# cvjena/semantic-embeddings

Hardware: AMD Instinct MI355X
Metric: retrieval_Mpairs_per_sec (higher is better)
Workload: dtype f32

## Files before the change

semantic-embeddings_amd/csrc/rank_rows.hip:

```cpp
#include "se_common.h"
#include <stdlib.h>
#include <atomic>
#include <type_traits>

namespace se {

constexpr int RK_THREADS = 512;
constexpr int RK_WAVES = RK_THREADS / WAVE;
constexpr int RK_ITEMS = 16;
constexpr int RK_TILE = RK_THREADS * RK_ITEMS;
constexpr int RK_WCHUNK = RK_TILE / RK_WAVES;
constexpr int RK_NB = 256;

struct RankLds {
    uint32_t gbase[4][RK_NB];
    uint32_t wcnt[RK_WAVES][RK_NB];
    uint32_t tile_start[RK_NB];
    uint32_t wave_tot[RK_WAVES];
    uint32_t tkeys[RK_TILE];
    uint32_t tidx[RK_TILE];
};

__device__ __forceinline__ uint32_t wave_excl_scan(uint32_t v, uint32_t &total)
{
// ... 131 lines not shown
                    }
                    if (valid) {
                        const int rnk = __popcll(peers & lt_mask);
                        const int npeers = __popcll(peers);
                        const uint32_t base = cur[dgt];
                        if (rnk == npeers - 1) cur[dgt] = base + (uint32_t)npeers;
                        L.tkeys[base + rnk] = key[s];
                        L.tidx[base + rnk] = idx[s];
                    }
                }
                wg_barrier();

#pragma unroll
                for (int j = 0; j < RK_ITEMS; j++) {
                    const int i = j * RK_THREADS + tid;
                    if (i < tcount) {
                        const uint32_t k = L.tkeys[i];
                        const uint32_t id = L.tidx[i];
                        const uint32_t d = (k >> shift) & 0xFF;
                        const uint32_t gpos = L.gbase[p][d] + ((uint32_t)i - L.tile_start[d]);
                        if (last) {
                            if (IDX64) ((int64_t *)rank)[row * ldr + gpos] = (int64_t)id;
                            else ((int32_t *)rank)[row * ldr + gpos] = (int32_t)id;
                        } else {
                            dk[gpos] = k;
                            di[gpos] = id;
                        }
                    }
                }
                wg_barrier();
                if (tid < RK_NB) L.gbase[p][tid] += my_total;
            }
        }
    }
}


constexpr int RR_THREADS = 512;
constexpr int RR_WAVES = RR_THREADS / WAVE;
constexpr int RR_SCAN_THREADS = 512;
constexpr int RR_SCAN_WAVES = RR_SCAN_THREADS / WAVE;
static_assert((53248 + RR_THREADS - 1) / RR_THREADS <= 104, "rows of up to 53,248 columns: 104 keys per thread");
constexpr int RR_G = 8;
constexpr int RR_MAX_N = 53248;

__device__ __forceinline__ void differ_mask(uint32_t d, uint32_t &lo, uint32_t &hi)
{
    lo = 0;
    hi = 0;
#pragma unroll
    for (int bb = 0; bb < 8; bb += 2) {
        uint32_t s0 = (uint32_t)__builtin_amdgcn_sbfe((int)d, bb, 1);
        uint32_t s1 = (uint32_t)__builtin_amdgcn_sbfe((int)d, bb + 1, 1);
        asm volatile("" : "+v"(s0), "+v"(s1));
        const uint64_t m0 = __ballot(s0 != 0), m1 = __ballot(s1 != 0);
        lo = __builtin_amdgcn_bitop3_b32(lo, (uint32_t)m0, s0, 0xF6);
        hi = __builtin_amdgcn_bitop3_b32(hi, (uint32_t)(m0 >> 32), s0, 0xF6);
        lo = __builtin_amdgcn_bitop3_b32(lo, (uint32_t)m1, s1, 0xF6);
        hi = __builtin_amdgcn_bitop3_b32(hi, (uint32_t)(m1 >> 32), s1, 0xF6);
    }
}

constexpr uint32_t RR_KEY_NAN = 0xFF900000u;
__device__ __forceinline__ uint32_t rr_pad_key(uint32_t lane) { return 0xFFA00000u + ((lane % 6u) << 20) + (lane << 11) + lane; }
__device__ __forceinline__ uint32_t rr_key(uint32_t u, bool pad, uint32_t pad_key)
{
    const uint32_t sx = (uint32_t)((int32_t)u >> 31);
    uint32_t k = __builtin_amdgcn_bitop3_b32(u, sx, 0x80000000u, 0x1E);
    k -= sx;
    const float f = __uint_as_float(u);
    k = (f != f) ? RR_KEY_NAN : k;
    return pad ? pad_key : k;
}

__device__ __forceinline__ int32_t rr_clamp_i32(int32_t x, int32_t lo, int32_t hi) { return min(max(x, lo), hi); }

template <typename T>
__device__ __forceinline__ void opaque(T &x) { asm volatile("" : "+v"(x)); }

__device__ __forceinline__ uint32_t lds_off(const void *p) { return (uint32_t)(uintptr_t)p; }
__device__ __forceinline__ void lds_wait() { asm volatile("s_waitcnt lgkmcnt(0)" ::: "memory"); }
__device__ __forceinline__ void lds_st16_lo(uint32_t addr, uint32_t v) { asm volatile("ds_write_b16 %0, %1" ::"v"(addr), "v"(v) : "memory"); }
__device__ __forceinline__ void lds_st16_hi(uint32_t addr, uint32_t v) { asm volatile("ds_write_b16_d16_hi %0, %1" ::"v"(addr), "v"(v) : "memory"); }
template <int OFF>
__device__ __forceinline__ void lds_ld16(uint32_t &dst, uint32_t addr) { asm volatile("ds_read_u16 %0, %1 offset:%2" : "=v"(dst) : "v"(addr), "n"(OFF) : "memory"); }
template <int K>
__device__ __forceinline__ void lds_wait_le(uint32_t &landed) { asm volatile("s_waitcnt lgkmcnt(%1)" : "+v"(landed) : "n"(K) : "memory"); }

constexpr int RR_RING = 12;
template <int ITEMS, bool HI, int I = 0>
struct RRRead {
    static __device__ __forceinline__ void run(uint32_t (&a)[ITEMS], uint32_t (&t)[RR_RING], uint32_t addr)
    {
        constexpr int D = RR_RING - 1;
        if constexpr (I < ITEMS) lds_ld16<I * WAVE * 2>(t[I % RR_RING], addr);
        if constexpr (I >= D) {
            constexpr int J = I - D;
            constexpr int newest = (I < ITEMS ? I : ITEMS - 1);
            lds_wait_le<newest - J>(t[J % RR_RING]);
            a[J] = __builtin_amdgcn_perm(t[J % RR_RING], a[J], HI ? 0x05040100u : 0x03020504u);
        }
        if constexpr (I + 1 < ITEMS + D) RRRead<ITEMS, HI, I + 1>::run(a, t, addr);
    }
};

template <int ITEMS, int V, int S0, int I = 0>
struct RRRankFinish {
    static __device__ __forceinline__ void run(uint32_t (&ir)[ITEMS], uint32_t (&key)[ITEMS], uint32_t (&rnk)[V], uint32_t (&base)[V])
    {
        lds_wait_le<2 * (V - 1 - I) + 1>(base[I]);
        ir[S0 + I] = (ir[S0 + I] & 0xFFFF0000u) | (base[I] + rnk[I]);
        opaque(ir[S0 + I]);
        opaque(key[S0 + I]);
        if constexpr (I + 1 < V) RRRankFinish<ITEMS, V, S0, I + 1>::run(ir, key, rnk, base);
    }
};

template <int ITEMS, int S0 = 0>
struct RRRank {
    static __device__ __forceinline__ void run(uint32_t (&ir)[ITEMS], uint32_t (&key)[ITEMS], int shift, int lane, uint32_t cb)
    {
        constexpr int V = (ITEMS - S0 < RR_G) ? (ITEMS - S0) : RR_G;
        static_assert(2 * V - 1 <= 15, "lgkmcnt counts to 15");
        uint32_t rnk[V], base[V];
#pragma unroll
        for (int g = 0; g < V; g++) {
            const uint32_t d = (key[S0 + g] >> shift) & 0xFFu;
            uint32_t dlo, dhi;
            differ_mask(d, dlo, dhi);
            rnk[g] = (uint32_t)lane - __builtin_amdgcn_mbcnt_hi(dhi, __builtin_amdgcn_mbcnt_lo(dlo, 0u));
            const uint32_t ca = cb + (d << 2);
            asm volatile("ds_read_b32 %0, %1" : "=v"(base[g]) : "v"(ca) : "memory");
            if (rnk[g] == 0) {
                const uint32_t np = 64u - (uint32_t)(__popc(dlo) + __popc(dhi));
                asm volatile("ds_add_u32 %0, %1" ::"v"(ca), "v"(np) : "memory");
            }
        }
        RRRankFinish<ITEMS, V, S0>::run(ir, key, rnk, base);
        __builtin_amdgcn_sched_barrier(0);
        if constexpr (S0 + V < ITEMS) RRRank<ITEMS, S0 + V>::run(ir, key, shift, lane, cb);
    }
};

typedef int rr_i32x4 __attribute__((ext_vector_type(4)));
typedef long long rr_i64x2 __attribute__((ext_vector_type(2)));
constexpr int RR_GH = 8;
constexpr int RR_HW_BITS = 11;
constexpr int RR_WIDE_WORDS = 2048;
constexpr uint32_t RR_TWO_SPAN = (1u << 24) - 3u;
constexpr int RR_TWO_OUT = 256;
constexpr int RR_IMG_RUN = 8;
constexpr int RR_IMG_WL = 3072;
constexpr int RR_IMG_MAX_ITEMS = 98;
constexpr uint32_t RR_IMG_NAN_PADHI = 0xFF0u;
template <int ITEMS, bool PEEL, int S = 0>
struct RRRankHW {
    static __device__ __forceinline__ void run(uint32_t (&ir)[ITEMS], uint32_t (&key)[ITEMS], uint32_t (&r)[RR_GH], uint32_t (&sh)[RR_GH],
                                               uint32_t (&grp)[RR_GH], uint32_t shift, uint32_t hshift, uint32_t wlo, uint32_t whi, uint32_t cb,
                                               int lane, bool peel)
    {
        constexpr int SLOT = S % RR_GH;
        uint32_t ca = 0, inc = 0, shv = 0, g = 0xFFFFFFFFu;
        uint64_t part = ~0ull;
        if constexpr (S < ITEMS) {
            const uint32_t w = __builtin_amdgcn_ubfe(key[S], shift, wlo);
            const uint32_t h = __builtin_amdgcn_ubfe(key[S], hshift, whi);
// ... 78 lines not shown
    constexpr int NB = 1 << BITS;
    constexpr int NPASS = (32 + BITS - 1) / BITS;
    constexpr int CNT_WORDS = HWORD ? NB / 2 : NB;
    constexpr bool WIDE = HWORD && ((size_t)RR_THREADS * ITEMS * sizeof(uint16_t) >= (size_t)RR_WAVES * RR_WIDE_WORDS * sizeof(uint32_t));
    constexpr bool IMG = WIDE && VAR == 3;
    constexpr bool RAWKEYS = IMG || (WIDE && VAR == 2);
    static_assert(VAR != 3 || (WIDE && ITEMS <= RR_IMG_MAX_ITEMS && !SEG), "image path: long-row instantiations with room for the tag plane");
    uint32_t *wcnt = reinterpret_cast<uint32_t *>(rr_raw);
    uint32_t *wave_tot = reinterpret_cast<uint32_t *>(rr_raw + rr_region0_bytes<ITEMS, HWORD, VAR>());
    uint16_t *xbuf = reinterpret_cast<uint16_t *>(wave_tot + 32);
    [[maybe_unused]] uint8_t *tagb = rr_raw;
    [[maybe_unused]] uint32_t *wlist = reinterpret_cast<uint32_t *>(rr_raw + (size_t)RR_THREADS * ITEMS + 32);
    [[maybe_unused]] uint32_t *ictl = wave_tot + 24;
    const int tid = threadIdx.x, lane = tid & 63, wave = tid >> 6;
    [[maybe_unused]] const int wave_s = __builtin_amdgcn_readfirstlane(wave);
    const int wpos0 = wave * (ITEMS * WAVE) + lane;
    const uint32_t xb = lds_off(xbuf);
    const uint32_t rb = xb + 2u * (uint32_t)wpos0;
#define RR_DST(IR) (xb + (((IR) & 0xFFFFu) << 1))
    auto row_ptr = [&](int64_t v) -> const float * {
        if constexpr (SEG) return pdist + (v >> seg.shift) * ldp + (v & ((1 << seg.shift) - 1)) * (int64_t)seg.seg_n;
        else return pdist + v * ldp;
    };
    auto row_len = [&](int64_t v) -> int {
        if constexpr (SEG) {
            const int rest = N - (int)(v & ((1 << seg.shift) - 1)) * seg.seg_n;
            return rest < seg.seg_n ? rest : seg.seg_n;
        } else return N;
    };
    uint32_t t_acc[12] = {0, 0, 0, 0, 0, 0, 0, 0, 0, 0, 0, 0}, t_last = PROF ? (uint32_t)__builtin_amdgcn_s_memtime() : 0;
#define RR_T(i) if constexpr (PROF) { const uint32_t now = (uint32_t)__builtin_amdgcn_s_memtime(); t_acc[i] += now - t_last; t_last = now; } else { asm volatile("" ::: "memory"); __builtin_amdgcn_sched_barrier(0); }

    uint32_t key[ITEMS], ir[ITEMS];
    __amdgpu_buffer_rsrc_t ld_rsrc;
    uint32_t ld_voff = 0;
    uint32_t ring[RR_RING];
#define RR_LOAD_ONE(DROW, WPOS, S, NN)                                                                               \
    {                                                                                                                 \
        if ((S) % 16 == 0) {                                                                                          \
            if ((S) == 0) {                                                                                           \
                ld_rsrc = __builtin_amdgcn_make_buffer_rsrc(const_cast<float *>(DROW), 0, (NN) * 4, 0x00020000);     \
                ld_voff = (uint32_t)(WPOS) * 4u;                                                                      \
            } else ld_voff += 4096u;                                                                                  \
            opaque(ld_voff);                                                                                          \
        }                                                                                                             \
        key[S] = (uint32_t)__builtin_amdgcn_raw_buffer_load_b32(ld_rsrc, (int)ld_voff + ((S) % 16) * 256, 0, 0);      \
    }
#define RR_CANON(NN)                                                                                                  \
    {                                                                                                                 \
        int wpos_ = wpos0;                                                                                            \
        opaque(wpos_);                                                                                                \
        const uint32_t pk_ = rr_pad_key((uint32_t)wpos_ & 63u);                                                       \
        _Pragma("unroll") for (int s = 0; s < ITEMS; s++) {                                                           \
            const int pos = wpos_ + s * WAVE;                                                                         \
            key[s] = rr_key(key[s], pos >= (NN), pk_ + (ITEMS <= 88 ? (uint32_t)((((s >> 3) & 7) << 17) | ((s & 7) << 6)) : 0u));  \
        }                                                                                                             \
    }
#define RR_PREFETCH_NEXT_ROW() RR_PREFETCH_NEXT_ROW_IF(end >= 32 && more)
#define RR_PREFETCH_NEXT_ROW_IF(COND) \
    if (COND) { \
                const char *nrow = (const char *)row_ptr(row + gridDim.x); \
                const uint32_t row_bytes = (uint32_t)row_len(row + gridDim.x) * 4u; \
                for (uint32_t off = (uint32_t)tid * 128u; off < row_bytes; off += RR_THREADS * 128u) \
                    asm volatile("global_load_dword %0, %1, off" : "=v"(pf_sink) : "v"(nrow + off) : "memory"); \
            }
#define RR_STREAM_PLANE(P, ROW)                                                                                       \
    {                                                                                                                 \
        uint16_t *pl = seg.planes + (P) * seg.plane_elems + (ROW) * (int64_t)(RR_THREADS * ITEMS);                    \
        int j = tid * 8;                                                                                              \
        opaque(j);                                                                                                    \
        _Pragma("unroll 2") for (; j < RR_THREADS * ITEMS; j += RR_THREADS * 8)                                       \
            *reinterpret_cast<uint4 *>(pl + j) = *reinterpret_cast<const uint4 *>(xbuf + j);                          \
    }
    constexpr int RR_PADS = ITEMS < 8 ? ITEMS : 8;
#define RR_PAD_LOOP(NROW, BODY)                                                                                       \
    {                                                                                                                 \
        const int first_pad_ = ((NROW) - wave_s * (ITEMS * WAVE)) >> 6;    \
        if (first_pad_ >= ITEMS - RR_PADS) {                                                                          \
            _Pragma("unroll") for (int s = ITEMS - RR_PADS; s < ITEMS; s++) { BODY }                                  \
        } else {                                                                                                      \
            _Pragma("unroll") for (int s = 0; s < ITEMS; s++) { BODY }                                                \
        }                                                                                                             \
    }
    if ((int64_t)blockIdx.x < Q) {
        const float *drow = row_ptr(blockIdx.x);
        const int n0 = row_len(blockIdx.x);
        int wpos = wpos0;
        opaque(wpos);
#pragma unroll
        for (int s = 0; s < ITEMS; s++) RR_LOAD_ONE(drow, wpos, s, n0)
        if constexpr (!RAWKEYS) RR_CANON(n0)
    }
    uint32_t pf_sink = 0;
    [[maybe_unused]] int img_level = 0;
    [[maybe_unused]] bool img_again = false;
    [[maybe_unused]] int img_skip0 = 0, img_pen0 = 0, img_skip1 = 0, img_pen1 = 0;
    for (int64_t row = blockIdx.x; row < Q;) {
        const bool more = row + gridDim.x < Q;
        [[maybe_unused]] const int n_next = row_len(more ? row + gridDim.x : row);
        constexpr bool SKIP_WAVES = HWORD && ITEMS <= 88;
        const bool wave_live = !SKIP_WAVES || wave * (ITEMS * WAVE) < row_len(row);
        bool two = false;
        [[maybe_unused]] int n_out = 0;
        if constexpr (IMG) {
            const int n_row = row_len(row);
            if (!img_again) {
                if (img_skip1 > 0) { img_level = 2; img_skip1--; }
                else if (img_skip0 > 0) { img_level = 1; img_skip0--; }
                else img_level = 0;
            }
            bool attempt = img_level < 2;
            uint32_t cbits = 0, base = 0;
            if (attempt) {
                uint32_t mb = 0;
#pragma unroll
                for (int s = 0; s + 1 < ITEMS; s += 2) mb = max(max(mb, key[s] & 0x7FFFFFFFu), key[s + 1] & 0x7FFFFFFFu);
                if constexpr (ITEMS & 1) mb = max(mb, key[ITEMS - 1] & 0x7FFFFFFFu);
#pragma unroll
                for (int off = 32; off > 0; off >>= 1) mb = max(mb, (uint32_t)__shfl_xor((int)mb, off, 64));
                if (lane == 0) wave_tot[wave] = mb;
                wg_barrier();
                if (tid == 0) { ictl[0] = 0; ictl[1] = 0; }
#pragma unroll
                for (int w = 0; w < RR_WAVES; w++) mb = max(mb, wave_tot[w]);
                mb = (uint32_t)__builtin_amdgcn_readfirstlane((int)mb);
                const uint32_t e = (mb >> 23) + ((mb & 0x7FFFFFu) > 0x400000u ? 1u : 0u) - (img_level == 0 ? 1u : 0u);
                two = mb >= 0x0D800000u && mb < 0x7E800000u;
                cbits = (e + 1u) << 23;
                base = e << 23;
            }
            if (two) {
                const float c = __uint_as_float(cbits);
                int wpos_ = wpos0;
                opaque(wpos_);
                const uint32_t pk_ = ((RR_IMG_NAN_PADHI + ((uint32_t)wpos_ & 15u)) << 20) | (((uint32_t)wpos_ & 63u) << 14);
                const uint32_t tb = lds_off(tagb) + (uint32_t)wpos_;
#pragma unroll
                for (int s = 0; s < ITEMS; s++) {
                    const uint32_t t = __float_as_uint(__uint_as_float(key[s]) + c);
                    const uint32_t q = (uint32_t)rr_clamp_i32(__builtin_elementwise_sub_sat((int32_t)t, (int32_t)base), 0, 0xFEFFFF);
                    asm volatile("ds_write_b8 %0, %1 offset:%2" ::"v"(tb), "v"(q), "n"(s * WAVE) : "memory");
                    key[s] = q << 8;
                }
                if (wave_s * (ITEMS * WAVE) + ITEMS * WAVE > n_row) {
                    RR_PAD_LOOP(n_row, key[s] = (wpos_ + s * WAVE >= n_row) ? pk_ : key[s];)
                }
            } else {
                RR_CANON(n_row)
            }
            RR_T(8)
        }
        if constexpr (WIDE && VAR == 2) {
            uint32_t *stat = wave_tot;
            uint2 *outl = reinterpret_cast<uint2 *>(wcnt);
            const int n_row = row_len(row);
            int32_t mxi = 0;
            uint32_t umx = 0;
#pragma unroll
            for (int s = 0; s + 1 < ITEMS; s += 2) {
                mxi = max(max(mxi, rr_clamp_i32((int32_t)key[s], 0, 0x7F800000)), rr_clamp_i32((int32_t)key[s + 1], 0, 0x7F800000));
                umx = max(max(umx, key[s]), key[s + 1]);
            }
            if constexpr (ITEMS & 1) { mxi = max(mxi, rr_clamp_i32((int32_t)key[ITEMS - 1], 0, 0x7F800000)); umx = max(umx, key[ITEMS - 1]); }
            mxi = umx > 0xFF800000u ? 0x7F800000 : mxi;
#pragma unroll
            for (int off = 32; off > 0; off >>= 1) mxi = max(mxi, __shfl_xor(mxi, off, 64));
            if (lane == 0) stat[wave] = (uint32_t)mxi;
            if (tid == 0) stat[2 * RR_WAVES] = 0;
            RR_T(9)
            wg_barrier();
            RR_T(10)
#pragma unroll
            for (int w = 0; w < RR_WAVES; w++) mxi = max(mxi, (int32_t)stat[w]);
            const int32_t kmax = __builtin_amdgcn_readfirstlane(mxi);
            const int32_t lo = kmax > (int32_t)RR_TWO_SPAN ? kmax - (int32_t)RR_TWO_SPAN : 1, lo1 = lo - 1;
            uint32_t below_l = 0;
            {
                int wpos = wpos0;
                opaque(wpos);
#pragma unroll
                for (int s = 0; s < ITEMS; s++) below_l += ((int32_t)key[s] < lo) ? 1u : 0u;
                if (wave_s * (ITEMS * WAVE) + ITEMS * WAVE > n_row) {
                    int32_t lo_b = lo;
                    opaque(lo_b);
// ... 92 lines not shown
                    ex += c;
                }
            }
            } else {
                const bool scanner = tid < RR_SCAN_THREADS;
                const int st = scanner ? tid : 0;
                uint32_t T0 = 0, T1 = 0, U0 = 0, U1 = 0;
#pragma unroll
                for (int w = 0; w < RR_WAVES; w++) {
                    const uint2 v = *reinterpret_cast<const uint2 *>(pcnt + w * pcw + 2 * st);
                    T0 += v.x; T1 += v.y;
                }
                if (wide) {
                    __builtin_amdgcn_sched_barrier(0);
#pragma unroll
                    for (int w = 0; w < RR_WAVES; w++) {
                        const uint2 v = *reinterpret_cast<const uint2 *>(pcnt + w * pcw + CNT_WORDS + 2 * st);
                        U0 += v.x; U1 += v.y;
                    }
                    __builtin_amdgcn_sched_barrier(0);
                }
                uint32_t wtot, wtot2 = 0, ex2 = 0;
                uint32_t ex = wave_excl_scan(T0 + T1, wtot);
                if (wide) ex2 = wave_excl_scan(U0 + U1, wtot2);
                if (scanner && lane == 63) { wave_tot[wave] = wtot; wave_tot[RR_SCAN_WAVES + wave] = wtot2; }
                wg_barrier();
                uint32_t all = 0, all2 = 0;
#pragma unroll
                for (int w = 0; w < RR_SCAN_WAVES; w++) {
                    const uint32_t wt = wave_tot[w], wt2 = wave_tot[RR_SCAN_WAVES + w];
                    all += wt; all2 += wt2;
                    ex += (w < wave) ? wt : 0u;
                    ex2 += (w < wave) ? wt2 : 0u;
                }
                ex2 += all;
                const uint32_t hi = (all + all2) << 16;
                ex += hi; ex2 += hi;
                if (scanner) {
                uint32_t s0 = ex, s1 = ex + T0;
#pragma unroll
                for (int w = 0; w < RR_WAVES; w++) {
                    uint2 *wp = reinterpret_cast<uint2 *>(pcnt + w * pcw + 2 * tid);
                    const uint2 v = *wp;
                    *wp = make_uint2(s0, s1);
                    s0 += v.x; s1 += v.y;
                }
                if (wide) {
                    __builtin_amdgcn_sched_barrier(0);
                    s0 = ex2; s1 = ex2 + U0;
#pragma unroll
                    for (int w = 0; w < RR_WAVES; w++) {
                        uint2 *wp = reinterpret_cast<uint2 *>(pcnt + w * pcw + CNT_WORDS + 2 * tid);
                        const uint2 v = *wp;
                        *wp = make_uint2(s0, s1);
                        s0 += v.x; s1 += v.y;
                    }
                }
                }
            }
            wg_barrier();
            RR_T(2)
            if (!(IMG && two)) { RR_PREFETCH_NEXT_ROW() }
            if (wave_live) {
#pragma unroll
            for (int s0 = 0; s0 < ITEMS; s0 += 8) {
                uint32_t first[8];
#pragma unroll
                for (int g = 0; g < 8; g++)
                    if (s0 + g < ITEMS) {
                        if constexpr (HWORD) first[g] = reinterpret_cast<const uint16_t *>(mycnt)[(__builtin_amdgcn_ubfe(key[s0 + g], (uint32_t)shift, wlo) << 1) | __builtin_amdgcn_ubfe(key[s0 + g], hshift, whi)];
                        else first[g] = mycnt[(key[s0 + g] >> shift) & 0xFFu];
                    }
#pragma unroll
                for (int g = 0; g < 8; g++)
                    if (s0 + g < ITEMS) {
                        ir[s0 + g] += first[g];
                        opaque(ir[s0 + g]);
                    }
                __builtin_amdgcn_sched_barrier(0);
            }
            }
            if (wide) wg_barrier();
            RR_T(3)
            if (wave_live) {
#pragma unroll
                for (int s = 0; s < ITEMS; s++) { opaque(ir[s]); lds_st16_hi(RR_DST(ir[s]), ir[s]); }
            }
            lds_wait();
            wg_barrier();
            RR_T(4)
            const bool last = end >= 32;
            if (last) {
                if constexpr (!SEG) break;
                else {
                    RR_STREAM_PLANE(0, row)
                    wg_barrier();
                }
            } else {
                if (wave_live) RRRead<ITEMS, true>::run(ir, ring, rb);
                lds_wait();
                wg_barrier();
            }
            RR_T(5)
            if (wave_live) {
#pragma unroll
                for (int s = 0; s < ITEMS; s++) { opaque(ir[s]); lds_st16_hi(RR_DST(ir[s]), key[s]); }
            }
            lds_wait();
            wg_barrier();
            if (SEG && last) {
                RR_STREAM_PLANE(1, row)
            } else {
                if (wave_live) RRRead<ITEMS, true>::run(key, ring, rb);
                lds_wait();
            }
            if (end < 16 || SEG) {
                wg_barrier();
                if (wave_live) {
#pragma unroll
                    for (int s = 0; s < ITEMS; s++) { opaque(ir[s]); lds_st16_lo(RR_DST(ir[s]), key[s]); }
                }
                lds_wait();
                wg_barrier();
                if (SEG && last) break;
                if (wave_live) RRRead<ITEMS, false>::run(key, ring, rb);
                lds_wait();
            }
            RR_T(6)
        }
#undef RR_DST
        if constexpr (WIDE && VAR == 2) {
            if (two && n_out > 1) {
                const uint2 *outl = reinterpret_cast<const uint2 *>(wcnt);
                if (tid < n_out) {
                    const uint2 me = outl[tid];
                    int r = 0;
                    for (int j = 0; j < n_out; j++) {
                        const uint2 o = outl[j];
                        r += (o.x < me.x || (o.x == me.x && o.y < me.y)) ? 1 : 0;
                    }
                    xbuf[r] = (uint16_t)me.y;
                }
                wg_barrier();
            }
        }
        [[maybe_unused]] bool img_fail = false;
        if constexpr (IMG) {
            const float *drow = row_ptr(more ? row + gridDim.x : row);
            int wpos = wpos0;
            opaque(wpos);
#pragma unroll
            for (int s = 0; s < ITEMS; s++) RR_LOAD_ONE(drow, wpos, s, n_next)
        }
        if constexpr (IMG) {
            if (two) {
                int n_row = row_len(row);
                int tsc = wave_s * WAVE + (int)__builtin_amdgcn_mbcnt_hi(~0u, __builtin_amdgcn_mbcnt_lo(~0u, 0u));
                opaque(n_row);
                opaque(tsc);
                const float *drow_cur = row_ptr(row);
                constexpr int NS = RR_THREADS * ITEMS;
                constexpr int NG = (NS / 8 + RR_THREADS - 1) / RR_THREADS;
                uint32_t S[NG];
                uint32_t nstart = 0;
                uint4 xg[NG];
                uint32_t nxg[NG];
#pragma unroll
                for (int g = 0; g < NG; g++) {
                    const int b0 = (tsc + RR_THREADS * g) * 8;
                    const int bs = b0 < n_row - 1 ? b0 : 0;
                    xg[g] = *reinterpret_cast<const uint4 *>(xbuf + bs);
                    nxg[g] = xbuf[bs + 8 < NS ? bs + 8 : bs];
                }
                constexpr int TD = 1;
                uint32_t t[TD + 1][9];
                auto tag_reads = [&](int g, uint32_t (&tt)[9]) {
                    const uint32_t xi[4] = {xg[g].x, xg[g].y, xg[g].z, xg[g].w};
#pragma unroll
                    for (int j = 0; j < 4; j++) {
                        tt[2 * j] = tagb[xi[j] & 0xFFFFu];
                        tt[2 * j + 1] = tagb[xi[j] >> 16];
                    }
                    tt[8] = tagb[nxg[g]];
                };
#pragma unroll
                for (int g = 0; g < TD && g < NG; g++) tag_reads(g, t[g % (TD + 1)]);
#pragma unroll
                for (int g = 0; g < NG; g++) {
                    if (g + TD < NG) tag_reads(g + TD, t[(g + TD) % (TD + 1)]);
                    const uint32_t (&tc)[9] = t[g % (TD + 1)];
                    const bool live = (tsc + RR_THREADS * g) * 8 < n_row - 1;
                    const uint32_t A = tc[0] | (tc[1] << 8) | (tc[2] << 16) | (tc[3] << 24), B = tc[4] | (tc[5] << 8) | (tc[6] << 16) | (tc[7] << 24);
                    const uint32_t zA = A ^ __builtin_amdgcn_alignbyte(B, A, 1), zB = B ^ __builtin_amdgcn_alignbyte(tc[8], B, 1);
                    const uint32_t uA = (zA & 0x7F7F7F7Fu) + 0x7F7F7F7Fu, uB = (zB & 0x7F7F7F7Fu) + 0x7F7F7F7Fu;
                    const uint32_t eA = __builtin_amdgcn_bitop3_b32(uA, zA, 0x80808080u, 0x02), eB = __builtin_amdgcn_bitop3_b32(uB, zB, 0x80808080u, 0x02);
                    S[g] = live ? ((eA >> 7) | (eB >> 3)) : 0u;
                    nstart += (uint32_t)__popc(S[g]);
                }
                uint32_t slot = 0;
                {
                    const uint32_t ca = lds_off(&ictl[0]);
                    asm volatile("ds_add_rtn_u32 %0, %1, %2\n\ts_waitcnt lgkmcnt(0)" : "=v"(slot) : "v"(ca), "v"(nstart) : "memory");
                }
#pragma unroll
                for (int g = 0; g < NG; g++) {
                    uint32_t st = S[g];
                    const int b0 = (tsc + RR_THREADS * g) * 8;
                    while (st) {
                        const int bit = __builtin_ctz(st);
                        st &= st - 1u;
                        const int pos = b0 + (bit & 4) + (bit >> 3);
                        if (slot < (uint32_t)RR_IMG_WL) wlist[slot] = pos < n_row - 1 ? (uint32_t)pos : 0xFFFFFFFFu;
                        slot++;
                    }
                }
                wg_barrier();
                const uint32_t nwork = ictl[0];
                img_fail = nwork > (uint32_t)RR_IMG_WL;
                RR_T(9)
                if (!img_fail) {
                    constexpr int GB = 2;
#pragma unroll 1
                    for (uint32_t e0 = 0; e0 < nwork; e0 += RR_THREADS * GB) {
                        uint32_t pp[GB], im[GB], ia[GB], ib[GB], ic[GB], id[GB], tm[GB], t0[GB], t2[GB], t3[GB], ka[GB], kb[GB], kc[GB];
#pragma unroll
                        for (int k = 0; k < GB; k++) {
                            const uint32_t e = e0 + (uint32_t)(k * RR_THREADS + tsc);
                            pp[k] = e < nwork ? wlist[e] : 0xFFFFFFFFu;
                        }
#pragma unroll
                        for (int k = 0; k < GB; k++) {
                            const uint32_t p = pp[k] != 0xFFFFFFFFu ? pp[k] : 0u;
                            im[k] = xbuf[p ? p - 1u : 0u]; ia[k] = xbuf[p]; ib[k] = xbuf[p + 1];
                            ic[k] = xbuf[p + 2 < (uint32_t)NS ? p + 2 : p]; id[k] = xbuf[p + 3 < (uint32_t)NS ? p + 3 : p];
                        }
#pragma unroll
                        for (int k = 0; k < GB; k++) { tm[k] = tagb[im[k]]; t0[k] = tagb[ia[k]]; t2[k] = tagb[ic[k]]; t3[k] = tagb[id[k]]; }
#pragma unroll
                        for (int k = 0; k < GB; k++) {
                            const bool mine = pp[k] != 0xFFFFFFFFu && !(pp[k] != 0u && tm[k] == t0[k]);
                            const bool three = mine && (int)pp[k] + 2 < n_row && t2[k] == t0[k];
                            ka[k] = kb[k] = kc[k] = 0u;
                            if (mine) {
                                ka[k] = __float_as_uint(drow_cur[ia[k]]);
                                kb[k] = __float_as_uint(drow_cur[ib[k]]);
                            }
                            if (three) kc[k] = __float_as_uint(drow_cur[ic[k]]);
                        }
#pragma unroll
                        for (int k = 0; k < GB; k++) {
                            if (pp[k] == 0xFFFFFFFFu) continue;
                            const uint32_t p = pp[k];
                            if (p != 0u && tm[k] == t0[k]) continue;
                            const bool three = (int)p + 2 < n_row && t2[k] == t0[k];
                            const bool more4 = three && (int)p + 3 < n_row && t3[k] == t0[k];
                            const uint32_t ca = rr_key(ka[k], false, 0u), cb = rr_key(kb[k], false, 0u), cc = rr_key(kc[k], false, 0u);
                            if (!three) {
                                if (ca > cb) { xbuf[p] = (uint16_t)ib[k]; xbuf[p + 1] = (uint16_t)ia[k]; }
                            } else if (!more4) {
                                const uint32_t ra = (cb < ca) + (cc < ca), rb = (ca <= cb) + (cc < cb), rc = (ca <= cc) + (cb <= cc);
                                if (ra != 0u || rb != 1u) {
                                    xbuf[p + ra] = (uint16_t)ia[k]; xbuf[p + rb] = (uint16_t)ib[k]; xbuf[p + rc] = (uint16_t)ic[k];
                                }
                            } else {
                                int len = 4;
                                while (len <= RR_IMG_RUN && (int)p + len < n_row && tagb[xbuf[p + len]] == t0[k]) len++;
                                if (len > RR_IMG_RUN) { ictl[1] = 1u; continue; }
                                uint32_t idx[RR_IMG_RUN], kk[RR_IMG_RUN];
#pragma unroll
                                for (int j = 0; j < RR_IMG_RUN; j++) idx[j] = xbuf[p + (uint32_t)(j < len ? j : 0)];
#pragma unroll
                                for (int j = 0; j < RR_IMG_RUN; j++) kk[j] = rr_key(__float_as_uint(drow_cur[idx[j]]), false, 0u);
#pragma unroll
                                for (int j = 0; j < RR_IMG_RUN; j++) {
                                    uint32_t r = 0;
#pragma unroll
                                    for (int i = 0; i < RR_IMG_RUN; i++)
                                        if (i != j) r += (i < len && (kk[i] < kk[j] || (kk[i] == kk[j] && i < j))) ? 1u : 0u;
                                    if (j < len) xbuf[p + r] = (uint16_t)idx[j];
                                }
                            }
                        }
                    }
                    wg_barrier();
                    img_fail = ictl[1] != 0u;
                }
                RR_T(10)
            }
        }
        if (!IMG || img_fail) {
            const float *drow = row_ptr((IMG && img_fail) ? row : (more ? row + gridDim.x : row));
            int wpos = wpos0;
            opaque(wpos);
#pragma unroll
            for (int s = 0; s < ITEMS; s++) RR_LOAD_ONE(drow, wpos, s, n_next)
        }
        if constexpr (IMG) {
#pragma unroll
            for (int s = 0; s < ITEMS; s++) opaque(key[s]);
            asm volatile("s_waitcnt vmcnt(0)" : "+v"(pf_sink) : : "memory");
        }
        int wt = tid;
// ... 117 lines not shown
    const int cols = N < 1024 ? N : 1024;
    uint32_t kk[3][4];
#pragma unroll
    for (int r = 0; r < 3; r++) {
        const int64_t row = (r == 0) ? 0 : (r == 1 ? Q / 2 : Q - 1);
        const float *drow = pdist + row * ldp;
#pragma unroll
        for (int u = 0; u < 4; u++) {
            const int i = threadIdx.x + 256 * u;
            kk[r][u] = canon_key(drow[(int64_t)(i < cols ? i : 0) * N / cols]);
        }
    }
#pragma unroll
    for (int r = 0; r < 3; r++) {
#pragma unroll
        for (int u = 0; u < 4; u++) {
            const int i = threadIdx.x + 256 * u;
            if (i >= cols) continue;
            const uint32_t k = kk[r][u];
            atomicAdd(&hist[k >> shift], 1u);
            if (k != 0xFFFFFFFFu) atomicMax(&row_max[r], k);
            if (i < 256 && atomicAdd(&hash_hist[((k ^ ((uint32_t)r * 0x3C6EF372u)) * 2654435761u) >> 20], 1u) != 0u) atomicAdd(&repeats, 1u);
        }
    }
    wg_barrier();
#pragma unroll
    for (int r = 0; r < 3; r++) {
        const uint32_t lo = row_max[r] > RR_TWO_SPAN ? row_max[r] - RR_TWO_SPAN : 0u;
#pragma unroll
        for (int u = 0; u < 4; u++)
            if (threadIdx.x + 256 * u < cols && kk[r][u] < lo) atomicAdd(&row_below[r], 1u);
    }
    uint32_t mine = 0;
    for (int i = threadIdx.x; i < NBIN; i += 256) mine = hist[i] > mine ? hist[i] : mine;
    atomicMax(&best, mine);
    wg_barrier();
    if (threadIdx.x == 0) {
        const bool two = (two_ok & 1) && row_below[0] <= 4 && row_below[1] <= 4 && row_below[2] <= 4;
        const bool skewed = 10u * best >= 3u * 3u * (uint32_t)cols;
        const bool distinct = repeats < 3u * 96u;
        *flag = (two && distinct) ? 2u : (skewed ? 1u : (((two_ok & 2) && distinct) ? 3u : 0u));
    }
}

struct Resident { hipError_t err; int64_t grid; };
static Resident rank_resident(const void *kern, size_t lds)
{
    hipError_t e = hipFuncSetAttribute(kern, hipFuncAttributeMaxDynamicSharedMemorySize, (int)lds);
    int dev = 0, occ = 0;
    hipDeviceProp_t prop;
    if (e == hipSuccess) e = hipGetDevice(&dev);
    if (e == hipSuccess) e = hipGetDeviceProperties(&prop, dev);
    if (e == hipSuccess) e = hipOccupancyMaxActiveBlocksPerMultiprocessor(&occ, kern, RR_THREADS, lds);
    if (e != hipSuccess) return {e, 0};
    return {hipSuccess, (int64_t)(prop.multiProcessorCount > 0 ? prop.multiProcessorCount : 256) * (occ > 0 ? occ : 1)};
}

template <int ITEMS, bool HW, int VAR>
static int launch_rank_reg_variant(const float *pdist, int64_t ldp, int64_t q, int n, void *rank, int idx64, int64_t ldr,
                                   const uint32_t *skew_flag, hipStream_t s)
{
    const size_t lds = rr_region0_bytes<ITEMS, HW, VAR>() + 32 * sizeof(uint32_t) + (size_t)RR_THREADS * ITEMS * sizeof(uint16_t);
    static_assert(rr_region0_bytes<ITEMS, HW, VAR>() + 32 * sizeof(uint32_t) + (size_t)RR_THREADS * ITEMS * sizeof(uint16_t) <= 160 * 1024, "LDS of one CU");
    static const bool profile = tuning_env("SE_RR_PROFILE") != nullptr;
    auto kern = (kTuning && profile) ? rank_rows_reg_kernel<ITEMS, kTuning && (ITEMS == 98), HW, VAR> : rank_rows_reg_kernel<ITEMS, false, HW, VAR>;
    static const Resident res = rank_resident((const void *)kern, lds);
    if (res.err != hipSuccess) return fail(SE_ERR_HIP, "se_rank_rows: kernel set-up failed: %s", hipGetErrorString(res.err));
    int64_t grid = res.grid;
    if (grid > q) grid = q;
    const size_t esz = rank_idx_bytes(idx64);
    const int vec_ok = ((((uintptr_t)rank) & 15) == 0) && ((ldr * esz) % 16 == 0);
    unsigned long long *prof = nullptr;
    if (profile && ITEMS == 98) {
        SE_HIP_CHECK(hipMalloc((void **)&prof, 36 * sizeof(unsigned long long)));
        SE_HIP_CHECK(hipMemsetAsync(prof, 0, 36 * sizeof(unsigned long long), s));
    }
    hipLaunchKernelGGL(kern, dim3((unsigned)grid), dim3(RR_THREADS), lds, s, pdist, ldp, q, n, rank, ldr, idx64, vec_ok, prof, skew_flag, RankSeg{0, 0, nullptr, 0});
    SE_LAUNCH_CHECK();
    if (prof) {
        unsigned long long h[36];
        SE_HIP_CHECK(hipStreamSynchronize(s));
        SE_HIP_CHECK(hipMemcpy(h, prof, sizeof(h), hipMemcpyDeviceToHost));
        SE_HIP_CHECK(hipFree(prof));
        static const char *names[12] = {"load", "rank", "scan", "dest", "idx-write", "idx-read", "key-exchange", "write-out", "image-map|window-map", "tag-scan|window-max", "repair|window-barrier-1", "window-count"};
        double tot = 0;
        for (int i = 0; i < 12; i++) tot += (double)h[i];
        if (tot > 0) {
            fprintf(stderr, "[se_rank_rows profile] ITEMS=%d hw=%d peel=%d grid=%lld:", ITEMS, (int)HW, VAR, (long long)grid);
            for (int i = 0; i < 12; i++) fprintf(stderr, " %s %.1f%%", names[i], 100.0 * (double)h[i] / tot);
            fprintf(stderr, "  (%.0f cycles per row; wave 0 of every workgroup, timestamps behind the phases' own barriers)", tot / (double)q);
            fprintf(stderr, "\n");
        }
    }
    return SE_OK;
}

template <int ITEMS>
static int launch_rank_reg(const float *pdist, int64_t ldp, int64_t q, int n, void *rank, int idx64, int64_t ldr, bool hw, void *scratch,
                           hipStream_t s)
{
    if (!hw) return launch_rank_reg_variant<ITEMS, false, 0>(pdist, ldp, q, n, rank, idx64, ldr, nullptr, s);
    constexpr bool wide = (size_t)RR_THREADS * ITEMS * sizeof(uint16_t) >= (size_t)RR_WAVES * RR_WIDE_WORDS * sizeof(uint32_t);
    constexpr bool two_ok = wide;
    constexpr bool img_ok = wide && ITEMS <= RR_IMG_MAX_ITEMS;
    static const char *force = tuning_env("SE_RANK_PEEL");
    if (force || !scratch) {
        if (force && force[0] == '1') return launch_rank_reg_variant<ITEMS, true, 1>(pdist, ldp, q, n, rank, idx64, ldr, nullptr, s);
        if (force && force[0] == '2' && two_ok) return launch_rank_reg_variant<ITEMS, true, two_ok ? 2 : 0>(pdist, ldp, q, n, rank, idx64, ldr, nullptr, s);
        if (force && force[0] == '3' && img_ok) return launch_rank_reg_variant<ITEMS, true, img_ok ? 3 : 0>(pdist, ldp, q, n, rank, idx64, ldr, nullptr, s);
        return launch_rank_reg_variant<ITEMS, true, 0>(pdist, ldp, q, n, rank, idx64, ldr, nullptr, s);
    }
    uint32_t *flag = (uint32_t *)scratch + 16;
    const int top_shift = wide ? 20 : 2 * RR_HW_BITS;
    hipLaunchKernelGGL(rank_skew_detect_kernel, dim3(1), dim3(256), 0, s, pdist, ldp, q, n, top_shift, (two_ok ? 1 : 0) | (img_ok ? 2 : 0), flag);
    SE_LAUNCH_CHECK();
    int rc = launch_rank_reg_variant<ITEMS, true, 0>(pdist, ldp, q, n, rank, idx64, ldr, flag, s);
    if (rc != SE_OK) return rc;
    rc = launch_rank_reg_variant<ITEMS, true, 1>(pdist, ldp, q, n, rank, idx64, ldr, flag, s);
    if (rc != SE_OK) return rc;
    if (two_ok) rc = launch_rank_reg_variant<ITEMS, true, two_ok ? 2 : 0>(pdist, ldp, q, n, rank, idx64, ldr, flag, s);
    if (rc != SE_OK || !img_ok) return rc;
    return launch_rank_reg_variant<ITEMS, true, img_ok ? 3 : 0>(pdist, ldp, q, n, rank, idx64, ldr, flag, s);
}

constexpr int RC_CAP = 1022;
constexpr int MG_THREADS = 256;
constexpr int MG_VT = 16;
constexpr int RUNS_MAX_SEG = 8;

struct MergeLevel {
    int run_n, N, pairs, tiles, tile;
    const uint16_t *planes; int64_t plane_elems; int cap;
    const uint32_t *in_key, *in_idx; int64_t ld;
};

template <bool PLANES>
__device__ __forceinline__ uint32_t level_key(const MergeLevel &L, int64_t r, int run, int i)
{
    if constexpr (PLANES) {
        const uint16_t *khi = L.planes + L.plane_elems + (r * (2 * L.pairs) + run) * (int64_t)L.cap, *klo = khi + L.plane_elems;
        return ((uint32_t)khi[i] << 16) | klo[i];
    } else return L.in_key[r * L.ld + (int64_t)run * L.run_n + i];
}
__device__ __forceinline__ int level_run_len(const MergeLevel &L, int run)
{
    const int64_t rest = (int64_t)L.N - (int64_t)run * L.run_n;
    return rest <= 0 ? 0 : (rest < L.run_n ? (int)rest : L.run_n);
}

template <bool PLANES>
__global__ __launch_bounds__(256) void rank_merge_partition_kernel(const MergeLevel L, int64_t rows, int32_t *__restrict__ splits)
{
    const int64_t g = (int64_t)blockIdx.x * 256 + threadIdx.x;
    if (g >= rows * L.pairs * (L.tiles + 1)) return;
    const int64_t rp = g / (L.tiles + 1);
    const int t = (int)(g - rp * (L.tiles + 1));
    const int64_t r = rp / L.pairs;
    const int p = (int)(rp - r * L.pairs);
    const int na = level_run_len(L, 2 * p), nb = level_run_len(L, 2 * p + 1);
    const int64_t d64 = (int64_t)t * L.tile;
    const int d = (int)(d64 < na + nb ? d64 : na + nb);
    int lo = d > nb ? d - nb : 0, hi = d < na ? d : na;
    while (lo < hi) {
        const int mid = (lo + hi) >> 1;
        if (level_key<PLANES>(L, r, 2 * p, mid) <= level_key<PLANES>(L, r, 2 * p + 1, d - 1 - mid)) lo = mid + 1;
        else hi = mid;
    }
// ... 605 lines not shown
```

Baseline: 227,300.

## Overlap next-row global loads with last-pass index scatter in image path

For the IMG variant without wave skipping, the final radix pass exits before the index scatter. The scatter of ranks into LDS is then fused with the prefetch loads of the next row, so global load latency overlaps the LDS stores, and the destination address is computed with a single mad instruction. It also removes a per-lane neighbour load by taking the next byte from the adjacent lane through DPP, and reworks the profiling timestamps. This adds control-flow complexity and depends on the lane-boundary handling being correct.

New measurement: 233,600 (median of 6 runs). 1.03x the previous value.

```diff
diff --git a/semantic-embeddings_amd/csrc/rank_rows.hip b/semantic-embeddings_amd/csrc/rank_rows.hip
--- a/semantic-embeddings_amd/csrc/rank_rows.hip
+++ b/semantic-embeddings_amd/csrc/rank_rows.hip
@@ -237,6 +237,12 @@
 __device__ __forceinline__ void lds_wait() { asm volatile("s_waitcnt lgkmcnt(0)" ::: "memory"); }
 __device__ __forceinline__ void lds_st16_lo(uint32_t addr, uint32_t v) { asm volatile("ds_write_b16 %0, %1" ::"v"(addr), "v"(v) : "memory"); }
 __device__ __forceinline__ void lds_st16_hi(uint32_t addr, uint32_t v) { asm volatile("ds_write_b16_d16_hi %0, %1" ::"v"(addr), "v"(v) : "memory"); }
+__device__ __forceinline__ uint32_t rr_dst_mad(uint32_t ir, uint32_t xb)
+{
+    uint32_t a;
+    asm("v_mad_u32_u16 %0, %1, 2, %2" : "=v"(a) : "v"(ir), "s"(xb));
+    return a;
+}
 template <int OFF>
 __device__ __forceinline__ void lds_ld16(uint32_t &dst, uint32_t addr) { asm volatile("ds_read_u16 %0, %1 offset:%2" : "=v"(dst) : "v"(addr), "n"(OFF) : "memory"); }
 template <int K>
@@ -481,6 +487,18 @@
             _Pragma("unroll") for (int s = 0; s < ITEMS; s++) { BODY }                                                \
         }                                                                                                             \
     }
+#define RR_IDX_SCATTER_IMG(AFTER_STORE)                                                                               \
+    {                                                                                                                 \
+        opaque(ir[0]);                                                                                                \
+        uint32_t a_ = rr_dst_mad(ir[0], xb);                                                                          \
+        _Pragma("unroll") for (int s = 0; s < ITEMS; s++) {                                                           \
+            uint32_t an_ = 0;                                                                                         \
+            if (s + 1 < ITEMS) { opaque(ir[s + 1]); an_ = rr_dst_mad(ir[s + 1], xb); }                                \
+            lds_st16_hi(a_, ir[s]);                                                                        \
+            AFTER_STORE                                                                                               \
+            a_ = an_;                                                                                                 \
+        }                                                                                                             \
+    }
     if ((int64_t)blockIdx.x < Q) {
         const float *drow = row_ptr(blockIdx.x);
         const int n0 = row_len(blockIdx.x);
@@ -499,6 +517,7 @@
         [[maybe_unused]] const int n_next = row_len(more ? row + gridDim.x : row);
         constexpr bool SKIP_WAVES = HWORD && ITEMS <= 88;
         const bool wave_live = !SKIP_WAVES || wave * (ITEMS * WAVE) < row_len(row);
+        constexpr bool LOAD_IN_SCATTER = IMG && !SKIP_WAVES;
         bool two = false;
         [[maybe_unused]] int n_out = 0;
         if constexpr (IMG) {
@@ -757,9 +776,16 @@
             }
             if (wide) wg_barrier();
             RR_T(3)
+            if constexpr (LOAD_IN_SCATTER) {
+                if (end >= 32) break;
+            }
             if (wave_live) {
-#pragma unroll
-                for (int s = 0; s < ITEMS; s++) { opaque(ir[s]); lds_st16_hi(RR_DST(ir[s]), ir[s]); }
+                if constexpr (LOAD_IN_SCATTER) {
+                    RR_IDX_SCATTER_IMG()
+                } else {
+#pragma unroll
+                    for (int s = 0; s < ITEMS; s++) { opaque(ir[s]); lds_st16_hi(RR_DST(ir[s]), ir[s]); }
+                }
             }
             lds_wait();
             wg_barrier();
@@ -824,8 +850,15 @@
             const float *drow = row_ptr(more ? row + gridDim.x : row);
             int wpos = wpos0;
             opaque(wpos);
-#pragma unroll
-            for (int s = 0; s < ITEMS; s++) RR_LOAD_ONE(drow, wpos, s, n_next)
+            if constexpr (LOAD_IN_SCATTER) {
+                RR_IDX_SCATTER_IMG(RR_LOAD_ONE(drow, wpos, s, n_next))
+                lds_wait();
+                wg_barrier();
+                RR_T(4)
+            } else {
+#pragma unroll
+                for (int s = 0; s < ITEMS; s++) RR_LOAD_ONE(drow, wpos, s, n_next)
+            }
         }
         if constexpr (IMG) {
             if (two) {
@@ -843,9 +876,9 @@
 #pragma unroll
                 for (int g = 0; g < NG; g++) {
                     const int b0 = (tsc + RR_THREADS * g) * 8;
-                    const int bs = b0 < n_row - 1 ? b0 : 0;
+                    const int bs = b0 < NS ? b0 : 0;
                     xg[g] = *reinterpret_cast<const uint4 *>(xbuf + bs);
-                    nxg[g] = xbuf[bs + 8 < NS ? bs + 8 : bs];
+                    nxg[g] = xbuf[(tsc & 63) == 63 ? (bs + 8 < NS ? bs + 8 : bs) : 0];
                 }
                 constexpr int TD = 1;
                 uint32_t t[TD + 1][9];
@@ -866,7 +899,8 @@
                     const uint32_t (&tc)[9] = t[g % (TD + 1)];
                     const bool live = (tsc + RR_THREADS * g) * 8 < n_row - 1;
                     const uint32_t A = tc[0] | (tc[1] << 8) | (tc[2] << 16) | (tc[3] << 24), B = tc[4] | (tc[5] << 8) | (tc[6] << 16) | (tc[7] << 24);
-                    const uint32_t zA = A ^ __builtin_amdgcn_alignbyte(B, A, 1), zB = B ^ __builtin_amdgcn_alignbyte(tc[8], B, 1);
+                    const uint32_t t8 = (uint32_t)__builtin_amdgcn_update_dpp((int)tc[8], (int)tc[0], 0x130, 0xF, 0xF, false);
+                    const uint32_t zA = A ^ __builtin_amdgcn_alignbyte(B, A, 1), zB = B ^ __builtin_amdgcn_alignbyte(t8, B, 1);
                     const uint32_t uA = (zA & 0x7F7F7F7Fu) + 0x7F7F7F7Fu, uB = (zB & 0x7F7F7F7Fu) + 0x7F7F7F7Fu;
                     const uint32_t eA = __builtin_amdgcn_bitop3_b32(uA, zA, 0x80808080u, 0x02), eB = __builtin_amdgcn_bitop3_b32(uB, zB, 0x80808080u, 0x02);
                     S[g] = live ? ((eA >> 7) | (eB >> 3)) : 0u;
@@ -889,10 +923,11 @@
                         slot++;
                     }
                 }
+                if constexpr (PROF) { RR_T(9) }
                 wg_barrier();
                 const uint32_t nwork = ictl[0];
                 img_fail = nwork > (uint32_t)RR_IMG_WL;
-                RR_T(9)
+                RR_T(11)
                 if (!img_fail) {
                     constexpr int GB = 2;
 #pragma unroll 1
@@ -1176,7 +1211,7 @@
         SE_HIP_CHECK(hipStreamSynchronize(s));
         SE_HIP_CHECK(hipMemcpy(h, prof, sizeof(h), hipMemcpyDeviceToHost));
         SE_HIP_CHECK(hipFree(prof));
-        static const char *names[12] = {"load", "rank", "scan", "dest", "idx-write", "idx-read", "key-exchange", "write-out", "image-map|window-map", "tag-scan|window-max", "repair|window-barrier-1", "window-count"};
+        static const char *names[12] = {"load", "rank", "scan", "dest", "idx-write", "idx-read", "key-exchange", "write-out", "image-map|window-map", "tag-scan|window-max", "repair|window-barrier-1", "window-count|scan-barrier"};
         double tot = 0;
         for (int i = 0; i < 12; i++) tot += (double)h[i];
         if (tot > 0) {
```
